# alibaba/euler

Measured on NVIDIA H100. Metric: sampled_edges_per_sec, higher is better.
Workload: dtype u64 ids / f32 weights+features (f64 CDF compare)

## Files before the change

euler_b200/csrc/capi.cu:

```cuda
#include <stdio.h>
#include <stdlib.h>
#include <string.h>

#include <algorithm>
#include <map>
#include <mutex>
#include <string>

#include "internal.h"

namespace eu {

__global__ void k_seed(EuRngState* rs, int n, unsigned long long seed0, const unsigned long long* seeds) {
  const int e = blockIdx.x * blockDim.x + threadIdx.x;
  if (e >= n) return;
  const unsigned long long seed = seeds ? seeds[e] : seed0 + (unsigned long long)e;
  EuRngState* r = rs + e;
  unsigned long long x = seed % 2147483647ull;
  r->x = x == 0 ? 1u : (uint32_t)x;
  r->x_prev = r->x;
  r->draws = 0;
  r->calls = 0;
  r->blocks_done = 0;
  r->key = seed * 0x9E3779B97F4A7C15ull;
}

template <typename T>
static int regrow(T** p, int64_t count) {
  if (*p) cudaFree(*p);
  *p = nullptr;
  void* q = nullptr;
  size_t bytes = (size_t)(count > 0 ? count : 1) * sizeof(T);
  cudaError_t e = cudaMalloc(&q, bytes);
  if (e != cudaSuccess) { set_error("cudaMalloc(%zu) -> %s", bytes, cudaGetErrorString(e)); return EU_ERR_CUDA; }
  *p = (T*)q;
  return EU_OK;
}

int refuse_growth_in_capture(eu_ctx* c, const char* what) {
  cudaStreamCaptureStatus st = cudaStreamCaptureStatusNone;
  if (cudaStreamIsCapturing(c->stream, &st) == cudaSuccess && st != cudaStreamCaptureStatusNone) {
    set_error("%s must grow while the ctx stream is being captured: run the op once (or call eu_ctx_reserve) before the capture", what);
    return EU_ERR_STATE;
  }
  cudaGetLastError();
  return EU_OK;
}

int ctx_reserve(eu_ctx* c, int64_t rows, int64_t table_slots) {
  int rc;
  if ((table_slots > c->tab_set_slots || rows > c->cap_rows) && (rc = refuse_growth_in_capture(c, "the sampling scratch"))) return rc;
  if (table_slots > c->tab_set_slots) {
    EU_CUDA(cudaStreamSynchronize(c->stream));
    const int64_t slots = table_slots + 64;
    if ((rc = regrow(&c->d_dedup, 2 * slots))) return rc;
    c->tab_set_slots = slots;
    for (int64_t off = 0; off < 2 * slots; off += (int64_t)1 << 20) {
      int64_t n = std::min<int64_t>((int64_t)1 << 20, 2 * slots - off);
      EU_CUDA(cudaMemset2DAsync(&c->d_dedup[off].key, sizeof(HashSlot), 0x00, 8, (size_t)n, c->stream));
      EU_CUDA(cudaMemset2DAsync(&c->d_dedup[off].row, sizeof(HashSlot), 0xFF, 8, (size_t)n, c->stream));
    }
  }
  if (rows <= c->cap_rows) return EU_OK;
  EU_CUDA(cudaStreamSynchronize(c->stream));
  if ((rc = regrow(&c->d_first, rows))) return rc;
  if ((rc = regrow(&c->d_rowof, rows))) return rc;
  if ((rc = regrow(&c->d_elig, rows))) return rc;
  if ((rc = regrow(&c->d_state, rows))) return rc;
  if ((rc = regrow(&c->d_emask, rows / 32 + 2))) return rc;
  if ((rc = regrow(&c->d_woff, rows / 32 + 2))) return rc;
  if ((rc = regrow(&c->d_blkpre, rows / 256 + 66))) return rc;
  if ((rc = regrow(&c->d_blkmul, rows / 256 + 66))) return rc;
  if ((rc = regrow(&c->d_live, rows))) return rc;
  if ((rc = regrow(&c->d_dup, rows))) return rc;
  if (!c->d_nlive && (rc = regrow(&c->d_nlive, 4))) return rc;
  if ((rc = regrow(&c->d_front[0], rows))) return rc;
  if ((rc = regrow(&c->d_front[1], rows))) return rc;
  c->cap_rows = rows;
  return EU_OK;
}

int ctx_misc(eu_ctx* c, int64_t bytes) {
  if (bytes <= c->misc_bytes) return EU_OK;
  if (int rc0 = refuse_growth_in_capture(c, "the op scratch")) return rc0;
  EU_CUDA(cudaStreamSynchronize(c->stream));
  char* p = (char*)c->d_misc;
  int rc = regrow(&p, bytes);
  c->d_misc = p;
  if (rc) { c->misc_bytes = 0; return rc; }
  c->misc_bytes = bytes;
  return EU_OK;
}

int agg_reserve(eu_ctx* c, int64_t rows, int64_t table_slots) {
  if (rows <= c->agg_rows && table_slots <= c->agg_slots) return EU_OK;
  int rc;
  if ((rc = refuse_growth_in_capture(c, "the aggregation scratch"))) return rc;
  EU_CUDA(cudaStreamSynchronize(c->stream));
  if (table_slots > c->agg_slots) {
    c->agg_slots = 0;
    if ((rc = regrow(&c->d_agg_tab, table_slots))) return rc;
    EU_CUDA(cudaMemsetAsync(c->d_agg_tab, 0, sizeof(unsigned long long) * (size_t)table_slots, c->stream));
    c->agg_slots = table_slots;
  }
  if (rows > c->agg_rows) {
    c->agg_rows = 0;
    if ((rc = regrow(&c->d_agg_src, rows))) return rc;
    if ((rc = regrow(&c->d_agg_rep, rows))) return rc;
    if ((rc = regrow(&c->d_agg_slot, rows))) return rc;
    if (!c->d_agg_nrep && (rc = regrow(&c->d_agg_nrep, 1))) return rc;
    c->agg_rows = rows;
  }
  return EU_OK;
}

static std::mutex g_default_mu;
static eu_graph* g_default_graph = nullptr;
static eu_ctx* g_default_ctx = nullptr;

}

using namespace eu;

extern "C" {

int eu_ctx_create(eu_graph* g, eu_rng_kind rng, uint64_t seed, void* stream, eu_ctx** out) {
  if (!g || !out || (rng != EU_RNG_MINSTD && rng != EU_RNG_PHILOX)) { set_error("eu_ctx_create: bad argument"); return EU_ERR_INVALID; }
  EU_CUDA(cudaSetDevice(g->device));
  eu_ctx* c = new eu_ctx();
  c->g = g; c->rng = rng; c->seed = seed; c->stream = (cudaStream_t)stream;
  cudaError_t e = cudaMalloc(&c->d_rng, sizeof(EuRngState));
  if (e != cudaSuccess) { set_error("cudaMalloc rng -> %s", cudaGetErrorString(e)); delete c; return EU_ERR_CUDA; }
  k_seed<<<1, 64, 0, c->stream>>>(c->d_rng, 1, seed, nullptr);
  g_launches++;
  *out = c;
  return EU_OK;
}

int eu_ctx_destroy(eu_ctx* c) {
  if (!c) return EU_OK;
  cudaSetDevice(c->g->device);
  cudaStreamSynchronize(c->stream);
  cudaFree(c->d_rng); cudaFree(c->d_dedup); cudaFree(c->d_first); cudaFree(c->d_rowof);
  cudaFree(c->d_elig); cudaFree(c->d_state); cudaFree(c->d_emask); cudaFree(c->d_woff); cudaFree(c->d_blkpre); cudaFree(c->d_blkmul); cudaFree(c->d_live); cudaFree(c->d_dup); cudaFree(c->d_nlive); cudaFree(c->d_front[0]); cudaFree(c->d_front[1]);
  cudaFree(c->d_misc); cudaFree(c->d_stage); cudaFree(c->d_walkv);
  cudaFree(c->d_agg_tab); cudaFree(c->d_agg_src); cudaFree(c->d_agg_rep); cudaFree(c->d_agg_slot); cudaFree(c->d_agg_nrep);
  for (int i = 0; i < 2; ++i) { if (c->aux[i]) cudaStreamDestroy(c->aux[i]); if (c->ev_join[i]) cudaEventDestroy(c->ev_join[i]); }
  if (c->ev_fork) cudaEventDestroy(c->ev_fork);
  if (c->h_pin) cudaFreeHost(c->h_pin);
  delete c;
  return EU_OK;
}

int eu_ctx_set_stream(eu_ctx* c, void* stream) {
  if (!c) { set_error("null ctx"); return EU_ERR_INVALID; }
  c->stream = (cudaStream_t)stream;
  return EU_OK;
}

int eu_ctx_seed(eu_ctx* c, uint64_t seed) {
  if (!c) { set_error("null ctx"); return EU_ERR_INVALID; }
  EU_CUDA(cudaSetDevice(c->g->device));
  c->seed = seed;
  k_seed<<<1, 64, 0, c->stream>>>(c->d_rng, c->n_eng, seed, nullptr);
  EU_LAUNCHED();
  return EU_OK;
}

int eu_ctx_set_engines(eu_ctx* c, int32_t n, const uint64_t* seeds) {
  if (!c || n < 1 || n > 64) { set_error("eu_ctx_set_engines: 1..64 engines"); return EU_ERR_INVALID; }
  EU_CUDA(cudaSetDevice(c->g->device));
  EU_CUDA(cudaStreamSynchronize(c->stream));
  EuRngState* r = nullptr;
  EU_CUDA(cudaMalloc(&r, sizeof(EuRngState) * n));
  unsigned long long* d_seeds = nullptr;
  if (seeds) {
    EU_CUDA(cudaMalloc(&d_seeds, sizeof(unsigned long long) * n));
    EU_CUDA(cudaMemcpy(d_seeds, seeds, sizeof(unsigned long long) * n, cudaMemcpyHostToDevice));
    c->seed = seeds[0];
  }
  cudaFree(c->d_rng);
  c->d_rng = r;
  c->n_eng = n;
  k_seed<<<1, 64, 0, c->stream>>>(c->d_rng, n, c->seed, d_seeds);
  EU_LAUNCHED();
  EU_CUDA(cudaStreamSynchronize(c->stream));
  if (d_seeds) cudaFree(d_seeds);
  return EU_OK;
}

int eu_ctx_reserve(eu_ctx* c, int64_t max_rows) {
  if (!c || max_rows < 0) { set_error("eu_ctx_reserve: bad argument"); return EU_ERR_INVALID; }
  EU_CUDA(cudaSetDevice(c->g->device));
  const int nb = c->n_eng;
  int rc = ctx_reserve(c, max_rows + 256 * nb, 4 * max_rows + 65 * nb);
  if (rc) return rc;
// ... 101 lines not shown
```

euler_b200/csrc/internal.h:

```cpp
#pragma once
#include <cuda_runtime.h>
#include <stdint.h>

#include <atomic>
#include <string>
#include <vector>

#include "../../include/euler_b200.h"
#include "common.cuh"

namespace eu {

void set_error(const char* fmt, ...);
extern std::atomic<uint64_t> g_launches;

#define EU_CUDA(call)                                                                    \
  do {                                                                                   \
    cudaError_t _e = (call);                                                             \
    if (_e != cudaSuccess) {                                                             \
      ::eu::set_error("%s:%d %s -> %s", __FILE__, __LINE__, #call, cudaGetErrorString(_e)); \
      return EU_ERR_CUDA;                                                                \
    }                                                                                    \
  } while (0)

// ... 29 lines not shown
  eu::DevGraph d{};
  std::vector<void*> allocs;
  int64_t hbm_bytes = 0;
  bool sampler_built = false;
  std::vector<eu::TypeSampler> samplers;
  std::vector<float> type_sums;
  std::vector<float> type_prob;
  std::vector<int32_t> type_alias;
  float type_fwc_sum = 0.f;
  float* d_type_prob = nullptr;
  int32_t* d_type_alias = nullptr;
  std::vector<int64_t> sampler_order;
  std::vector<std::string> edge_type_names, node_type_names;
  std::vector<std::string> dense_feature_names;
  std::vector<std::string> sparse_feature_names, binary_feature_names;
  std::vector<uint64_t> u64_slot_max;
  eu::DevEdges e{};
  bool edges_set = false;
  struct EdgeSampler { int64_t n = 0; const int64_t* order = nullptr; const float* prob = nullptr; const int32_t* alias = nullptr; float fwc_sum = 0.f; };
  std::vector<EdgeSampler> edge_samplers;
  std::vector<std::string> edge_dense_names, edge_sparse_names, edge_binary_names;
  bool labels_built = false;
  std::vector<std::string> labels;
  int32_t* d_label_ptr = nullptr;
  unsigned long long* d_label_ids = nullptr;

  template <typename T>
  int alloc(T** p, int64_t count) {
    size_t bytes = (size_t)(count > 0 ? count : 1) * sizeof(T);
    bytes = (bytes + 255) & ~(size_t)255;
    void* q = nullptr;
    cudaError_t e = cudaMalloc(&q, bytes);
    if (e != cudaSuccess) {
      eu::set_error("cudaMalloc(%zu) -> %s", bytes, cudaGetErrorString(e));
      return EU_ERR_CUDA;
    }
    allocs.push_back(q);
    hbm_bytes += (int64_t)bytes;
    *p = (T*)q;
    return EU_OK;
  }
};

struct EuRngState {
  uint32_t x;
  uint32_t x_prev;
  unsigned long long draws;
  unsigned long long calls;
  unsigned int blocks_done;
  unsigned int pad2;
  unsigned long long key;
};

struct eu_ctx {
  eu_graph* g = nullptr;
  eu_rng_kind rng = EU_RNG_MINSTD;
  uint64_t seed = 0;
  cudaStream_t stream = nullptr;
  EuRngState* d_rng = nullptr;
  int n_eng = 1;
  int64_t cap_rows = 0;
  eu::HashSlot* d_dedup = nullptr;
  int64_t tab_set_slots = 0;
  int32_t* d_first = nullptr;
  int64_t* d_rowof = nullptr;
  uint8_t* d_elig = nullptr;
  uint32_t* d_state = nullptr;
  uint32_t* d_emask = nullptr;
  uint32_t* d_woff = nullptr;
  uint32_t* d_blkpre = nullptr;
  uint32_t* d_blkmul = nullptr;
  int32_t* d_live = nullptr;
  int32_t* d_dup = nullptr;
  unsigned int* d_nlive = nullptr;
  unsigned long long* d_front[2] = {nullptr, nullptr};
  int64_t agg_rows = 0, agg_slots = 0;
  unsigned long long* d_agg_tab = nullptr;
  int32_t* d_agg_src = nullptr;
  int32_t* d_agg_rep = nullptr;
  uint32_t* d_agg_slot = nullptr;
  unsigned int* d_agg_nrep = nullptr;
  void* d_misc = nullptr;
  int64_t misc_bytes = 0;
  float* d_walkv = nullptr;
  long long walkv_cap = 0;
  cudaStream_t aux[2] = {nullptr, nullptr};
  cudaEvent_t ev_fork = nullptr, ev_join[2] = {nullptr, nullptr};
  void* h_pin = nullptr;
  int64_t pin_bytes = 0;
  void* d_stage = nullptr;
  int64_t stage_bytes = 0;
  bool prof = false;
  struct ProfRec { const char* name; int64_t rows; cudaEvent_t e0, e1; };
  std::vector<ProfRec> prof_recs;
};

struct EuProfScope {
  eu_ctx* c; size_t idx;
  EuProfScope(eu_ctx* c_, const char* name, int64_t rows) : c(c_), idx((size_t)-1) {
    if (!c->prof) return;
    eu_ctx::ProfRec r{name, rows, nullptr, nullptr};
    cudaEventCreate(&r.e0); cudaEventCreate(&r.e1);
    cudaEventRecord(r.e0, c->stream);
    c->prof_recs.push_back(r);
    idx = c->prof_recs.size() - 1;
  }
  ~EuProfScope() { if (idx != (size_t)-1) cudaEventRecord(c->prof_recs[idx].e1, c->stream); }
};

namespace eu {
static constexpr int64_t kRepeatMinRows = (int64_t)1 << 17;
int ctx_reserve(eu_ctx* c, int64_t rows, int64_t table_slots);
int64_t hop_scratch_rows(int nb, int64_t rows_b);
int64_t hop_table_slots(int nb, int64_t rows_b);
int64_t hop_table_cap(int64_t rows_b);
int ctx_misc(eu_ctx* c, int64_t bytes);
inline size_t a256(size_t b) { return (b + 255) & ~(size_t)255; }
struct EdgeOrder;
// ... 22 lines not shown
```

euler_b200/csrc/sample.cu:

```cuda
#include <algorithm>

#include <stdlib.h>

#include "internal.h"

namespace eu {

struct ETypes {
  int32_t K;
  int32_t v[EU_MAX_ETYPES];
};

struct Geom {
  int32_t nb;
  int32_t nblk_b;
  int64_t rows_b;
  int64_t rows_pad;
  int64_t cap_b;
  const int32_t* rows_act;
};

__global__ void k_dedup_insert(HashSlot* tabs, Geom gm, const unsigned long long* __restrict__ seeds) {
  const int b = blockIdx.y;
  const int64_t li = blockIdx.x * (int64_t)blockDim.x + threadIdx.x;
// ... 5 lines not shown
  if ((threadIdx.x & 31) != __ffs(peers) - 1) return;
  dedup_insert_one(tabs + (int64_t)b * (gm.cap_b + 1), (unsigned long long)dedup_cap_eff(gm.cap_b, gm.rows_act, b) - 1, id, li);
}

__device__ __forceinline__ int64_t dedup_first(const HashSlot* tab, unsigned long long mask,
                                               unsigned long long id) {
  unsigned long long tag = id + 1;
  if (tag == 0ull) return (int64_t)tab[mask + 1].row;
  unsigned long long h = mix64(id) & mask;
  while (true) {
    const ulonglong2 s = *reinterpret_cast<const ulonglong2*>(tab + h);
    if (s.x == tag) return (int64_t)s.y;
    h = (h + 1) & mask;
  }
}

__device__ __forceinline__ float grp_cum_at(const DevGraph& g, int64_t row, int32_t t) {
  if (g.grp_cum) return __ldg(g.grp_cum + row * g.T + t);
  const int64_t b = g.grp_ptr[row], e = g.grp_ptr[row + 1];
  return e > b ? __ldg(g.cum_w + e - 1) : 0.f;
}

__device__ __forceinline__ bool row_eligible(const DevGraph& g, int64_t row, const ETypes& et, int mode) {
  if (row < 0) return false;
  const int32_t T = g.T;
  if (mode == 0) {
    int32_t t = et.v[0];
    if (t < 0 || t >= T) return false;
    return g.grp_ptr[row * T + t + 1] > g.grp_ptr[row * T + t];
  }
  if (mode == 1) {
    float s = 0.f;
    for (int32_t i = 0; i < et.K; ++i) {
      int32_t t = et.v[i];
      if (t < 0 || t >= T) return false;
      float pre = t > 0 ? grp_cum_at(g, row, t - 1) : 0.f;
      s = __fadd_rn(s, __fsub_rn(grp_cum_at(g, row, t), pre));
    }
    return s != 0.f;
  }
  return grp_cum_at(g, row, T - 1) != 0.f;
}

struct PrepOut {
  unsigned long long* eng_ids;
  long long* out_ids;
  float* out_w;
  int32_t* out_t;
  int32_t count;
  long long default_node;
  HashSlot* next_tabs;
  int64_t next_cap_b;
  int32_t* live;
  unsigned int* n_live;
  int32_t* dup;
  unsigned int* n_dup;
};

static constexpr int kPrepBlock = 256;

__global__ void __launch_bounds__(kPrepBlock) k_prepare(DevGraph g, const HashSlot* tabs, Geom gm,
                                                        const unsigned long long* __restrict__ seeds,
                                                        ETypes et, int mode, uint32_t F, unsigned long long draws_per_row,
                                                        int32_t* first, int64_t* rowof, uint32_t* emask, uint32_t* wmul,
                                                        uint32_t* blkpre, uint32_t* blkmul, EuRngState* rngs, PrepOut po) {
  __shared__ uint32_t s_w[kPrepBlock / 32];
  __shared__ uint32_t s_l[kPrepBlock / 32];
  __shared__ uint32_t s_d[kPrepBlock / 32];
  __shared__ uint32_t s_z[kPrepBlock / 32];
  __shared__ bool s_last;
  const int b = blockIdx.y;
  const int64_t li = blockIdx.x * (int64_t)kPrepBlock + threadIdx.x;
  const int64_t ii = b * gm.rows_pad + li;
  const int lane = threadIdx.x & 31, wid = threadIdx.x >> 5;
  EuRngState* rng = rngs + b;
  bool e = false;
  bool own = false;
  bool dflt = false;
  const int64_t rows_here = gm.rows_act ? (int64_t)gm.rows_act[b] : gm.rows_b;
  const uint32_t nblk_act = (uint32_t)max((int64_t)1, (rows_here + kPrepBlock - 1) / kPrepBlock);
  if (blockIdx.x >= nblk_act) return;
  if (li < rows_here) {
    const int64_t w = b * gm.rows_b + li;
    const unsigned long long id = seeds[w];
    const int64_t f = tabs ? dedup_first(tabs + (int64_t)b * (gm.cap_b + 1), (unsigned long long)dedup_cap_eff(gm.cap_b, gm.rows_act, b) - 1, id) : li;
    first[ii] = (int32_t)f;
    const int64_t row = lookup_row(g, id);
    own = row_eligible(g, row, et, mode);
    e = own && f == li;
    dflt = !own;
    if (own) rowof[ii] = row;
  }
  const uint32_t zm = __ballot_sync(0xffffffffu, dflt);
  if (zm) {
    const int64_t ob = (b * gm.rows_b + (li - lane)) * (int64_t)po.count;
    const uint32_t n = 32u * (uint32_t)po.count;
    for (uint32_t k = lane; k < n; k += 32) {
      if (!((zm >> (k / (uint32_t)po.count)) & 1u)) continue;
      if (po.eng_ids) po.eng_ids[ob + k] = 0ull;
      if (po.out_ids) { po.out_ids[ob + k] = po.default_node; po.out_w[ob + k] = 0.f; po.out_t[ob + k] = -1; }
    }
  }
  const uint32_t m = __ballot_sync(0xffffffffu, e);
  const uint32_t lm = po.dup ? m : __ballot_sync(0xffffffffu, own);
  const uint32_t dm = po.dup ? __ballot_sync(0xffffffffu, own && !e) : 0u;
  if (lane == 0) { s_w[wid] = __popc(m); s_l[wid] = __popc(lm); s_d[wid] = __popc(dm); s_z[wid] = zm; }
  __syncthreads();
  if (lane == 0) {
    uint32_t off = 0;
    for (int k = 0; k < wid; ++k) off += s_w[k];
    emask[ii >> 5] = m;
    uint32_t fp = 1, fb = F;
    for (; off; off >>= 1) { if (off & 1) fp = modmul(fp, fb); fb = modmul(fb, fb); }
    wmul[ii >> 5] = fp;
  }
  uint32_t* bp = blkpre + (int64_t)b * gm.nblk_b;
  if (threadIdx.x == 0) {
    uint32_t tot = 0, lt = 0, dt = 0;
    for (int k = 0; k < kPrepBlock / 32; ++k) {
      tot += s_w[k];
      const uint32_t l = s_l[k], d = s_d[k];
      s_l[k] = lt; s_d[k] = dt;
      lt += l; dt += d;
    }
    const uint32_t lbase = lt ? atomicAdd(po.n_live, lt) : 0u, dbase = dt ? atomicAdd(po.n_dup, dt) : 0u;
    for (int k = 0; k < kPrepBlock / 32; ++k) { s_l[k] += lbase; s_d[k] += dbase; }
    if (po.next_tabs)
      for (int k = 0; k < kPrepBlock / 32; ++k)
        if (s_z[k]) {
          const int64_t lz = blockIdx.x * (int64_t)kPrepBlock + k * 32 + (__ffs(s_z[k]) - 1);
          dedup_insert_one(po.next_tabs + (int64_t)b * (po.next_cap_b + 1), (unsigned long long)po.next_cap_b - 1, 0ull,
                           lz * (int64_t)po.count);
          break;
        }
    bp[blockIdx.x] = tot;
    __threadfence();
    s_last = atomicAdd(&rng->blocks_done, 1u) == nblk_act - 1;
  }
  __syncthreads();
  {
    const uint32_t below = (1u << lane) - 1u;
    if (e || (own && !po.dup)) po.live[s_l[wid] + __popc(lm & below)] = (int32_t)(b * gm.rows_b + li);
    else if (own) po.dup[s_d[wid] + __popc(dm & below)] = (int32_t)(b * gm.rows_b + li);
  }
  if (!s_last) return;
  __threadfence();
  __shared__ uint32_t s_scan[kPrepBlock];
  uint32_t carry = 0;
  for (uint32_t base = 0; base < nblk_act; base += kPrepBlock) {
    const uint32_t k = base + threadIdx.x;
    const uint32_t v = k < nblk_act ? __ldcg(bp + k) : 0u;
    s_scan[threadIdx.x] = v;
    __syncthreads();
    for (int off = 1; off < kPrepBlock; off <<= 1) {
      uint32_t t = threadIdx.x >= off ? s_scan[threadIdx.x - off] : 0u;
      __syncthreads();
      s_scan[threadIdx.x] += t;
      __syncthreads();
    }
    if (k < nblk_act) {
      uint32_t pre = carry + s_scan[threadIdx.x] - v;
      bp[k] = pre;
      uint32_t fp = 1, fb = F;
      for (; pre; pre >>= 1) { if (pre & 1) fp = modmul(fp, fb); fb = modmul(fb, fb); }
      blkmul[(int64_t)b * gm.nblk_b + k] = fp;
    }
    carry += s_scan[kPrepBlock - 1];
    __syncthreads();
  }
  if (threadIdx.x == 0) {
    uint32_t fp = 1, base = F;
    for (uint32_t t = carry; t; t >>= 1) { if (t & 1) fp = modmul(fp, base); base = modmul(base, base); }
    rng->x_prev = rng->x;
    rng->x = modmul(rng->x, fp);
    rng->draws += (unsigned long long)carry * draws_per_row;
    rng->blocks_done = 0;
  }
}

__global__ void __launch_bounds__(1024) k_state_scan(const uint8_t* __restrict__ elig, int64_t rows,
                                                     uint32_t F, unsigned long long draws_per_row,
                                                     uint32_t* state, EuRngState* rng) {
  __shared__ uint32_t s_part[1024];
  __shared__ uint32_t s_cnt[1024];
  const int t = threadIdx.x;
  const int64_t chunk = (rows + 1023) / 1024;
  const int64_t b = t * chunk, e = min(rows, b + chunk);
  uint32_t prod = 1, cnt = 0;
  for (int64_t i = b; i < e; ++i)
    if (elig[i]) { prod = modmul(prod, F); ++cnt; }
  s_part[t] = prod;
  s_cnt[t] = cnt;
  __syncthreads();
  for (int off = 1; off < 1024; off <<= 1) {
    uint32_t v = 1, c = 0;
    if (t >= off) { v = s_part[t - off]; c = s_cnt[t - off]; }
    __syncthreads();
    if (t >= off) { s_part[t] = modmul(s_part[t], v); s_cnt[t] += c; }
    __syncthreads();
  }
  const uint32_t x0 = rng->x;
  uint32_t run = modmul(x0, t > 0 ? s_part[t - 1] : 1u);
  for (int64_t i = b; i < e; ++i) {
    state[i] = run;
    if (elig[i]) run = modmul(run, F);
  }
  __syncthreads();
  if (t == 1023) {
    rng->x = modmul(x0, s_part[1023]);
    rng->draws += (unsigned long long)s_cnt[1023] * draws_per_row;
  }
}

struct SampleArgs {
  const unsigned long long* seeds;
  Geom gm;
  int32_t count;
  long long default_node;
  ETypes et;
  int mode;
  const int32_t* live;
  const unsigned int* n_live;
  const int32_t* first;
  const int64_t* rowof;
  const uint32_t* emask;
  const uint32_t* wmul;
  const uint32_t* blkmul;
  uint32_t F;
  uint32_t lanepow[32];
  uint32_t stride;
  int sg_log;
  int stage;
  HashSlot* clear_tab;
  int64_t clear_n;
  HashSlot* next_tabs;
  int64_t next_cap_b;
  unsigned long long key;
  const EuRngState* rngs;
  unsigned long long* eng_ids;
  long long* out_ids;
  float* out_w;
  int32_t* out_t;
};

__device__ __forceinline__ int lane_upper_bound(float c, int lo, int hi, float thr, unsigned gmask, int SG) {
#pragma unroll
  for (int it = 0; it < 5; ++it) {
    int mid = (lo + hi) >> 1;
    float v = __shfl_sync(gmask, c, mid, SG);
    bool go = lo < hi;
    bool gt = v >= thr;
    hi = (go && gt) ? mid : hi;
    lo = (go && !gt) ? mid + 1 : lo;
  }
  return lo;
}

template <bool PHILOX, int CTAS>
__global__ void __launch_bounds__(256, CTAS) k_sample(DevGraph g, SampleArgs a) {
  const int lane = threadIdx.x & 31;
  const int64_t gtid = blockIdx.x * (int64_t)blockDim.x + threadIdx.x;
  __shared__ uint32_t s_lanepow[32];
  __shared__ uint32_t s_fpow[32];
  constexpr int kStageF = 16;
  __shared__ __align__(128) float s_stage[256 * kStageF];
  __shared__ __align__(8) unsigned long long s_bar[32];
  const int SG = 1 << a.sg_log;
  const int sl = lane & (SG - 1);
  const unsigned gmask = SG == 32 ? 0xffffffffu : (((1u << SG) - 1u) << (lane - sl));
  const bool can_stage = a.sg_log >= 3 && a.stage;
  unsigned long long* const bar = &s_bar[can_stage ? (threadIdx.x >> a.sg_log) : 0];
  float* const sm = s_stage + (threadIdx.x - sl) * kStageF;
  const int64_t capg = (int64_t)SG * kStageF;
  uint32_t phase = 0;
  if (can_stage && sl == 0) mbar_init(bar, 1);
  if (!PHILOX && threadIdx.x < 32) {
    s_lanepow[threadIdx.x] = a.lanepow[threadIdx.x];
    uint32_t fp = 1, fb = a.F;
    for (uint32_t e = threadIdx.x; e; e >>= 1) { if (e & 1) fp = modmul(fp, fb); fb = modmul(fb, fb); }
    s_fpow[threadIdx.x] = fp;
  }
  fence_mbar_init();
  __syncthreads();
  if (!PHILOX) {
    if (!a.gm.rows_act) {
      for (int64_t s = gtid; s < a.clear_n; s += (int64_t)gridDim.x * blockDim.x) { a.clear_tab[s].key = 0; a.clear_tab[s].row = kEmptyRow; }
    } else if (a.clear_n) {
      for (int b = 0; b < a.gm.nb; ++b) {
        HashSlot* tab = a.clear_tab + (int64_t)b * (a.gm.cap_b + 1);
        const int64_t n = dedup_cap_eff(a.gm.cap_b, a.gm.rows_act, b) + 1;
        for (int64_t s = gtid; s < n; s += (int64_t)gridDim.x * blockDim.x) { tab[s].key = 0; tab[s].row = kEmptyRow; }
      }
    }
  }
  const int32_t count = a.count;
  const int32_t T = g.T;
  const int64_t total = PHILOX ? a.gm.nb * a.gm.rows_b : (int64_t)__ldg(a.n_live);
  const int64_t qstride = (((int64_t)gridDim.x * blockDim.x) >> 5) << (5 - a.sg_log);
  const uint32_t upd = a.mode == 0 ? 1u : 2u;
  const uint32_t stride = a.stride;

  for (int64_t q = ((gtid >> 5) << (5 - a.sg_log)) + (lane >> a.sg_log); q < total; q += qstride) {
    const int64_t w = PHILOX ? q : (int64_t)a.live[q];
    const int bidx = (int)(w / a.gm.rows_b);
    const int64_t li = w - bidx * a.gm.rows_b;
    if (PHILOX && a.gm.rows_act && li >= a.gm.rows_act[bidx]) continue;
    const int64_t obase = w * (int64_t)count;
    const EuRngState* rng = a.rngs + bidx;
    HashSlot* ntab = a.next_tabs ? a.next_tabs + (int64_t)bidx * (a.next_cap_b + 1) : nullptr;
    const unsigned long long nmask = (unsigned long long)a.next_cap_b - 1;
    const int64_t nbase = li * (int64_t)count;

    int64_t row;
    bool ok;
    uint32_t st = 0;
    unsigned long long seed_id = 0;
    if (PHILOX) {
      seed_id = a.seeds[w];
      row = lookup_row(g, seed_id);
      ok = row_eligible(g, row, a.et, a.mode);
    } else {
      const int64_t ib = bidx * a.gm.rows_pad;
      const int32_t f = a.first[ib + li];
      const uint32_t m = a.emask[(ib + f) >> 5];
      ok = (m >> (f & 31)) & 1u;
      if (ok) {
        row = a.rowof[ib + li];
        st = modmul(modmul(rng->x_prev, a.blkmul[(int64_t)bidx * a.gm.nblk_b + f / kPrepBlock]),
                    modmul(a.wmul[(ib + f) >> 5], s_fpow[__popc(m & ((1u << (f & 31)) - 1u))]));
      } else {
        row = -1;
      }
    }
    if (!ok) {
      for (int32_t j = sl; j < count; j += SG) {
        if (a.eng_ids) a.eng_ids[obase + j] = 0ull;
        if (a.out_ids) { a.out_ids[obase + j] = a.default_node; a.out_w[obase + j] = 0.f; a.out_t[obase + j] = -1; }
      }
      if (!PHILOX && ntab && sl == 0) dedup_insert_one(ntab, nmask, 0ull, nbase);
      continue;
    }

    const int64_t* gp = g.grp_ptr + row * T;
    const int64_t base = gp[0];
    const int64_t rlen = gp[T] - base;
    const bool small_row = rlen <= SG;
    float c = __int_as_float(0x7f800000);
    if (small_row && sl < rlen) c = __ldg(g.cum_w + base + sl);
    const int mis = (int)((reinterpret_cast<uintptr_t>(g.cum_w + base) & 15u) >> 2);
    const bool mid_row = can_stage && !small_row && rlen + mis <= capg;
    if (mid_row && sl == 0) {
      const uint32_t bytes = (uint32_t)((((rlen + mis) << 2) + 15) & ~15ll);
      fence_proxy_async_smem();
      mbar_arrive_expect_tx(bar, bytes);
      bulk_copy_g2s(sm, g.cum_w + base - mis, bytes, bar);
    }
    const float* const srow = sm + mis;

    int64_t gb = 0, ge = 0;
    float lim_b = 0.f, lim_e = 0.f;
    if (a.mode == 0) {
      const int32_t t = a.et.v[0];
      gb = gp[t];
      ge = gp[t + 1] - 1;
      lim_b = gb == base ? 0.f : __ldg(g.cum_w + gb - 1);
      lim_e = __ldg(g.cum_w + ge);
    }
    float tc = __int_as_float(0x7f800000);
    int ntc = 0;
    if (a.mode == 1) {
      ntc = a.et.K;
      float sum = 0.f, mine = 0.f;
      for (int32_t i = 0; i < ntc; ++i) {
        int32_t t = a.et.v[i];
        float pre = t > 0 ? grp_cum_at(g, row, t - 1) : 0.f;
        sum = __fadd_rn(sum, __fsub_rn(grp_cum_at(g, row, t), pre));
        if (i == sl) mine = sum;
      }
      if (sl < ntc) tc = mine;
    } else if (a.mode == 2) {
      ntc = T;
      if (sl < T) tc = grp_cum_at(g, row, sl);
    }
    const float tc_end = __shfl_sync(gmask, tc, ntc > 0 ? ntc - 1 : 0, SG);

    uint32_t x = 0;
    if (!PHILOX) x = modmul(st, s_lanepow[sl]);
    const uint32_t salt = PHILOX ? (uint32_t)rng->calls : 0u;
    const unsigned long long pkey = PHILOX ? a.key ^ rng->key : 0ull;

    if (mid_row) {
      const long long t0 = clock64();
      while (!mbar_try_wait(bar, phase))
        if (clock64() - t0 > 4000000000LL) __trap();
      phase ^= 1u;
    }
    bool keep = true;
    bool bad = false;
    for (int32_t j0 = 0; j0 < count; j0 += SG) {
      const int32_t j = j0 + sl;
      const bool active = j < count;
      double u_t = 0.0, u_n = 0.0;
      if (PHILOX) {
        philox_uniform2(seed_id, (uint32_t)j, salt, pkey, u_t, u_n);
      } else {
        uint32_t xs = x;
        if (upd == 2u) u_t = minstd_uniform(xs);
        u_n = minstd_uniform(xs);
        x = modmul(x, stride);
      }
      int32_t etype = a.mode == 0 ? a.et.v[0] : 0;
      int64_t b = gb, e = ge;
      float lb = lim_b, le = lim_e;
      if (a.mode != 0) {
        const float tt = gt_threshold(pick_r(u_t, 0.f, tc_end));
        int k = lane_upper_bound(tc, 0, ntc - 1, tt, gmask, SG);
        etype = a.mode == 1 ? a.et.v[k] : k;
        b = gp[etype];
        e = gp[etype + 1] - 1;
        if (e < b) {
          bad = bad || active;
          b = base; e = base;
        }
        lb = b == base ? 0.f : __ldg(g.cum_w + b - 1);
        le = __ldg(g.cum_w + e);
      }
      const float thr = gt_threshold(pick_r(u_n, lb, le));
      int64_t m;
      float wgt;
      if (small_row) {
        int li2 = lane_upper_bound(c, (int)(b - base), (int)(e - base), thr, gmask, SG);
        float hi_v = __shfl_sync(gmask, c, li2, SG);
        float lo_v = __shfl_sync(gmask, c, li2 > 0 ? li2 - 1 : 0, SG);
        m = base + li2;
        wgt = __fsub_rn(hi_v, li2 > 0 ? lo_v : 0.f);
      } else if (mid_row) {
        int lo = (int)(b - base), hi = (int)(e - base);
        while (lo < hi) {
          const int mid = (lo + hi) >> 1;
          if (srow[mid] >= thr) hi = mid; else lo = mid + 1;
// ... 150 lines not shown

static Geom make_geom(int nb, int64_t rows_b) {
  Geom gm{};
  gm.nb = nb;
  gm.rows_b = rows_b;
  gm.nblk_b = (int32_t)ceil_div(rows_b > 0 ? rows_b : 1, kPrepBlock);
  gm.rows_pad = (int64_t)gm.nblk_b * kPrepBlock;
  gm.cap_b = 64;
  while (gm.cap_b < rows_b * 2) gm.cap_b <<= 1;
  gm.rows_act = nullptr;
  return gm;
}

__global__ void k_ragged_stats(const long long* __restrict__ ptr, int64_t rows, long long* __restrict__ stats) {
  long long mx = 0;
  for (int64_t i = blockIdx.x * (int64_t)blockDim.x + threadIdx.x; i < rows; i += (int64_t)gridDim.x * blockDim.x)
    mx = max(mx, __ldg(ptr + i + 1) - __ldg(ptr + i));
  if (mx > 0) atomicMax(stats + 1, mx);
  if (blockIdx.x == 0 && threadIdx.x == 0) stats[0] = __ldg(ptr + rows);
}

int64_t hop_scratch_rows(int nb, int64_t rows_b) { return make_geom(nb, rows_b).rows_pad * nb; }
int64_t hop_table_slots(int nb, int64_t rows_b) { return (make_geom(nb, rows_b).cap_b + 1) * nb; }
int64_t hop_table_cap(int64_t rows_b) { return make_geom(1, rows_b).cap_b; }

int hop(eu_ctx* c, const unsigned long long* seeds, int64_t rows_b, const int32_t* etypes,
        int32_t K, int32_t count, int64_t default_node, unsigned long long* eng_ids,
        int64_t* out_ids, float* out_w, int32_t* out_t, int hop_index, bool pre_inserted, bool insert_next, int nb,
        const int32_t* rows_act, bool raw) {
  const int64_t rows = rows_b * nb;
  if (rows == 0 || count == 0) return EU_OK;
  if (nb < 1 || nb > c->n_eng) { set_error("hop: %d batches but the ctx has %d engines", nb, c->n_eng); return EU_ERR_INVALID; }
  const DevGraph& d = c->g->d;
  SampleArgs a{};
  int rc = classify(d, etypes, K, &a.et, &a.mode);
  if (rc) return rc;
  if (a.mode != 0 && d.T > 32) { set_error("T > 32 unsupported"); return EU_ERR_UNSUPPORTED; }
  cudaStream_t s = c->stream;
  Geom gm = make_geom(nb, rows_b);
  gm.rows_act = rows_act;
  a.seeds = seeds; a.gm = gm; a.count = count; a.default_node = default_node;
  a.eng_ids = eng_ids; a.out_ids = (long long*)out_ids; a.out_w = out_w; a.out_t = out_t;
  a.rngs = c->d_rng;
  {
    int need = std::min<int>(count, 32);
    if (a.mode == 1) need = std::max<int>(need, std::min<int>(a.et.K, 32));
    if (a.mode == 2) need = std::max<int>(need, std::min<int>(d.T, 32));
    a.sg_log = 0;
    while ((1 << a.sg_log) < need) ++a.sg_log;
  }
  static const int stage_rows = [] { const char* e = getenv("EU_SAMPLE_STAGE"); return e ? (atoi(e) != 0 ? 1 : 0) : 1; }();
  a.stage = stage_rows;
  static const int grid_ctas = [] { const char* e = getenv("EU_SAMPLE_CTAS"); return e ? std::min(8, std::max(1, atoi(e))) : 8; }();
  const int ctas = grid_ctas == 6 ? 6 : 8;
  const unsigned blocks = (unsigned)std::min<int64_t>(ceil_div(ceil_div(rows * 32, (int64_t)(32 >> a.sg_log)), 256), kSMs * grid_ctas);
  if (c->rng == EU_RNG_PHILOX) {
    a.key = c->seed;
    { EuProfScope ps(c, "k_sample<philox>", rows); if (ctas == 6) k_sample<true, 6><<<blocks, 256, 0, s>>>(d, a); else k_sample<true, 8><<<blocks, 256, 0, s>>>(d, a); }
    EU_LAUNCHED();
    k_bump_calls<<<1, 64, 0, s>>>(c->d_rng, nb);
    EU_LAUNCHED();
    return EU_OK;
  }
  if (rows >= ((int64_t)1 << 31) || nb > 64) { set_error("rows >= 2^31 or more than 64 batches"); return EU_ERR_UNSUPPORTED; }
  const Geom ng = make_geom(nb, rows_b * count);
  const bool chain = insert_next && eng_ids;
  rc = ctx_reserve(c, std::max(gm.rows_pad, chain ? ng.rows_pad : 0) * nb, (std::max(gm.cap_b, chain ? ng.cap_b : 0) + 1) * nb);
  if (rc) return rc;
  const int tb = kPrepBlock;
  HashSlot* tabs = c->d_dedup + (hop_index & 1) * c->tab_set_slots;
  HashSlot* ntabs = c->d_dedup + ((hop_index + 1) & 1) * c->tab_set_slots;
  if (raw && (pre_inserted || insert_next)) { set_error("hop: raw mode does not chain"); return EU_ERR_INVALID; }
  if (!pre_inserted && !raw) {
    EuProfScope ps(c, "k_dedup_insert", rows);
    k_dedup_insert<<<dim3((unsigned)ceil_div(gm.rows_b, tb), (unsigned)nb), tb, 0, s>>>(tabs, gm, seeds);
    EU_LAUNCHED();
  }
  const unsigned long long upr = (unsigned long long)count * (a.mode == 0 ? 1 : 2);
  const uint32_t F = modpow_a(2ull * upr);
  { EuProfScope ps(c, "k_prepare", rows);
    PrepOut po{};
    po.eng_ids = eng_ids; po.out_ids = (long long*)out_ids; po.out_w = out_w; po.out_t = out_t;
    po.count = count; po.default_node = default_node;
    if (chain) { po.next_tabs = ntabs; po.next_cap_b = ng.cap_b; }
    po.live = c->d_live; po.n_live = c->d_nlive;
    if (!raw && rows >= kRepeatMinRows) { po.dup = c->d_dup; po.n_dup = c->d_nlive + 1; }
    EU_CUDA(cudaMemsetAsync(c->d_nlive, 0, 2 * sizeof(unsigned int), s));
    k_prepare<<<dim3((unsigned)gm.nblk_b, (unsigned)nb), tb, 0, s>>>(d, raw ? nullptr : tabs, gm, seeds, a.et, a.mode, F, upr, c->d_first,
                                                                     c->d_rowof, c->d_emask, c->d_woff, c->d_blkpre, c->d_blkmul,
                                                                     c->d_rng, po); }
  EU_LAUNCHED();
  a.first = c->d_first; a.rowof = c->d_rowof; a.emask = c->d_emask; a.wmul = c->d_woff; a.blkmul = c->d_blkmul;
  a.live = c->d_live; a.n_live = c->d_nlive;
  a.F = F;
  const uint32_t upd = a.mode == 0 ? 1u : 2u;
  for (uint32_t k = 0; k < 32; ++k) a.lanepow[k] = modpow_a(2ull * upd * k);
  a.stride = modpow_a(2ull * upd * (unsigned long long)(1u << a.sg_log));
  a.clear_tab = tabs;
  a.clear_n = raw ? 0 : (gm.cap_b + 1) * nb;
  if (chain) {
    a.next_tabs = ntabs;
    a.next_cap_b = ng.cap_b;
  }
  { EuProfScope ps(c, "k_sample<minstd>", rows); if (ctas == 6) k_sample<false, 6><<<blocks, 256, 0, s>>>(d, a); else k_sample<false, 8><<<blocks, 256, 0, s>>>(d, a); }
  EU_LAUNCHED();
  if (!raw && rows >= kRepeatMinRows) {
    EuProfScope ps(c, "k_copy_dups", rows);
    k_copy_dups<<<blocks, 256, 0, s>>>(gm, count, a.sg_log, c->d_dup, c->d_nlive + 1, c->d_first, eng_ids, (long long*)out_ids, out_w, out_t);
    EU_LAUNCHED();
  }
  return EU_OK;
}

}

using namespace eu;

extern "C" {

int eu_sample_neighbor(eu_ctx* c, const int64_t* nodes, int64_t B, const int32_t* etypes, int32_t K,
                       int32_t count, int64_t default_node, int64_t* out_ids, float* out_w,
                       int32_t* out_t) {
  if (!c || B < 0 || count < 0 || (K > 0 && !etypes)) { set_error("eu_sample_neighbor: bad argument"); return EU_ERR_INVALID; }
  EU_CUDA(cudaSetDevice(c->g->device));
  return hop(c, (const unsigned long long*)nodes, B, etypes, K, count, default_node, nullptr, out_ids, out_w, out_t, 0, false, false, 1);
}

int eu_sample_neighbor_raw(eu_ctx* c, const int64_t* nodes, int64_t B, const int32_t* etypes, int32_t K,
                           int32_t count, int64_t* out_ids, float* out_w, int32_t* out_t) {
  if (!c || B < 0 || count < 0 || (K > 0 && !etypes)) { set_error("eu_sample_neighbor_raw: bad argument"); return EU_ERR_INVALID; }
  EU_CUDA(cudaSetDevice(c->g->device));
  if (c->rng != EU_RNG_MINSTD) { set_error("eu_sample_neighbor_raw: exact-RNG contexts only (philox rows are keyed on the node id: duplicates would repeat)"); return EU_ERR_UNSUPPORTED; }
  return hop(c, (const unsigned long long*)nodes, B, etypes, K, count, 0, nullptr, out_ids, out_w, out_t, 0, false, false, 1,
             nullptr, true);
}

int eu_sample_fanout_batched(eu_ctx* c, const int64_t* nodes, int32_t nb, int64_t B, const int32_t* etypes, int32_t K,
                             const int32_t* counts, int32_t L, int64_t default_node, int64_t* const* out_ids,
                             float* const* out_w, int32_t* const* out_t) {
  if (!c || nb < 1 || B < 0 || L < 0 || !counts || (K > 0 && !etypes)) { set_error("eu_sample_fanout: bad argument"); return EU_ERR_INVALID; }
  EU_CUDA(cudaSetDevice(c->g->device));
  if (nb > c->n_eng) { set_error("eu_sample_fanout_batched: %d batches but the ctx has %d engines (eu_ctx_set_engines)", nb, c->n_eng); return EU_ERR_INVALID; }
  for (int l = 0; l < L; ++l)
    if (counts[l] < 0) { set_error("negative count"); return EU_ERR_INVALID; }
  for (int l = 0; l < L; ++l)
    if (counts[l] == 0) { L = l; break; }
  if (B == 0) return EU_OK;
  int64_t rows_b = B, max_rows = hop_scratch_rows(nb, B), max_slots = hop_table_slots(nb, B), widest = B * nb;
  for (int l = 0; l < L; ++l) {
    rows_b *= counts[l];
    if (l + 1 < L) { max_rows = std::max(max_rows, hop_scratch_rows(nb, rows_b)); max_slots = std::max(max_slots, hop_table_slots(nb, rows_b)); }
    widest = std::max(widest, rows_b * nb);
  }
  int rc = ctx_reserve(c, std::max(max_rows, widest), max_slots);
  if (rc) return rc;
  const unsigned long long* seeds = (const unsigned long long*)nodes;
  rows_b = B;
// ... 126 lines not shown
```

Baseline: 5.540 billion.

## Precompute per-live-row records in prepare and prefetch them in sampler

k_prepare now writes a compact LiveRow record (row base, length, type-range or row id, and a per-row RNG multiplier) next to each live index. The sampler then reads this record instead of re-reading grp_ptr, first, emask and wmul, and it prefetches the next iteration's record. The block multiplier now has x_prev folded in. The sampler's launch bound drops to 3 CTAs per SM with a matching smaller grid, which allows more registers per thread. The cost is extra prepare work (a serial prefix loop and modpow per eligible row) and a larger scratch buffer. Non-eligible rows are no longer written as defaults in the minstd path, so that path must be covered elsewhere.

Result: faster. 6.058 billion (median of 6 runs) (+9.4%).

```diff
diff --git a/euler_b200/csrc/capi.cu b/euler_b200/csrc/capi.cu
--- a/euler_b200/csrc/capi.cu
+++ b/euler_b200/csrc/capi.cu
@@ -64,7 +64,7 @@
   if (rows <= c->cap_rows) return EU_OK;
   EU_CUDA(cudaStreamSynchronize(c->stream));
   if ((rc = regrow(&c->d_first, rows))) return rc;
-  if ((rc = regrow(&c->d_rowof, rows))) return rc;
+  if ((rc = regrow(&c->d_liverec, rows))) return rc;
   if ((rc = regrow(&c->d_elig, rows))) return rc;
   if ((rc = regrow(&c->d_state, rows))) return rc;
   if ((rc = regrow(&c->d_emask, rows / 32 + 2))) return rc;
@@ -141,7 +141,7 @@
   if (!c) return EU_OK;
   cudaSetDevice(c->g->device);
   cudaStreamSynchronize(c->stream);
-  cudaFree(c->d_rng); cudaFree(c->d_dedup); cudaFree(c->d_first); cudaFree(c->d_rowof);
+  cudaFree(c->d_rng); cudaFree(c->d_dedup); cudaFree(c->d_first); cudaFree(c->d_liverec);
   cudaFree(c->d_elig); cudaFree(c->d_state); cudaFree(c->d_emask); cudaFree(c->d_woff); cudaFree(c->d_blkpre); cudaFree(c->d_blkmul); cudaFree(c->d_live); cudaFree(c->d_dup); cudaFree(c->d_nlive); cudaFree(c->d_front[0]); cudaFree(c->d_front[1]);
   cudaFree(c->d_misc); cudaFree(c->d_stage); cudaFree(c->d_walkv);
   cudaFree(c->d_agg_tab); cudaFree(c->d_agg_src); cudaFree(c->d_agg_rep); cudaFree(c->d_agg_slot); cudaFree(c->d_agg_nrep);
diff --git a/euler_b200/csrc/internal.h b/euler_b200/csrc/internal.h
--- a/euler_b200/csrc/internal.h
+++ b/euler_b200/csrc/internal.h
@@ -105,6 +105,15 @@
   unsigned long long key;
 };
 
+namespace eu {
+struct LiveRow {
+  int64_t base;
+  int64_t aux;
+  int32_t rlen;
+  uint32_t lmul;
+};
+}
+
 struct eu_ctx {
   eu_graph* g = nullptr;
   eu_rng_kind rng = EU_RNG_MINSTD;
@@ -116,7 +125,7 @@
   eu::HashSlot* d_dedup = nullptr;
   int64_t tab_set_slots = 0;
   int32_t* d_first = nullptr;
-  int64_t* d_rowof = nullptr;
+  eu::LiveRow* d_liverec = nullptr;
   uint8_t* d_elig = nullptr;
   uint32_t* d_state = nullptr;
   uint32_t* d_emask = nullptr;
diff --git a/euler_b200/csrc/sample.cu b/euler_b200/csrc/sample.cu
--- a/euler_b200/csrc/sample.cu
+++ b/euler_b200/csrc/sample.cu
@@ -81,6 +81,7 @@
   HashSlot* next_tabs;
   int64_t next_cap_b;
   int32_t* live;
+  LiveRow* rec;
   unsigned int* n_live;
   int32_t* dup;
   unsigned int* n_dup;
@@ -91,7 +92,7 @@
 __global__ void __launch_bounds__(kPrepBlock) k_prepare(DevGraph g, const HashSlot* tabs, Geom gm,
                                                         const unsigned long long* __restrict__ seeds,
                                                         ETypes et, int mode, uint32_t F, unsigned long long draws_per_row,
-                                                        int32_t* first, int64_t* rowof, uint32_t* emask, uint32_t* wmul,
+                                                        int32_t* first, uint32_t* emask, uint32_t* wmul,
                                                         uint32_t* blkpre, uint32_t* blkmul, EuRngState* rngs, PrepOut po) {
   __shared__ uint32_t s_w[kPrepBlock / 32];
   __shared__ uint32_t s_l[kPrepBlock / 32];
@@ -106,6 +107,7 @@
   bool e = false;
   bool own = false;
   bool dflt = false;
+  LiveRow rec{};
   const int64_t rows_here = gm.rows_act ? (int64_t)gm.rows_act[b] : gm.rows_b;
   const uint32_t nblk_act = (uint32_t)max((int64_t)1, (rows_here + kPrepBlock - 1) / kPrepBlock);
   if (blockIdx.x >= nblk_act) return;
@@ -118,7 +120,17 @@
     own = row_eligible(g, row, et, mode);
     e = own && f == li;
     dflt = !own;
-    if (own) rowof[ii] = row;
+    if (own) {
+      const int64_t* gp = g.grp_ptr + row * g.T;
+      rec.base = gp[0];
+      rec.rlen = (int32_t)(gp[g.T] - rec.base);
+      if (mode == 0) {
+        const int32_t t = et.v[0];
+        rec.aux = (int64_t)(uint32_t)(gp[t] - rec.base) | ((gp[t + 1] - 1 - rec.base) << 32);
+      } else {
+        rec.aux = row;
+      }
+    }
   }
   const uint32_t zm = __ballot_sync(0xffffffffu, dflt);
   if (zm) {
@@ -169,12 +181,23 @@
   __syncthreads();
   {
     const uint32_t below = (1u << lane) - 1u;
-    if (e || (own && !po.dup)) po.live[s_l[wid] + __popc(lm & below)] = (int32_t)(b * gm.rows_b + li);
-    else if (own) po.dup[s_d[wid] + __popc(dm & below)] = (int32_t)(b * gm.rows_b + li);
+    if (e || (own && !po.dup)) {
+      const uint32_t at = s_l[wid] + __popc(lm & below);
+      po.live[at] = (int32_t)(b * gm.rows_b + li);
+      if (e) {
+        uint32_t pos = __popc(m & below);
+        for (int k = 0; k < wid; ++k) pos += s_w[k];
+        uint32_t fp = 1, fb = F;
+        for (; pos; pos >>= 1) { if (pos & 1) fp = modmul(fp, fb); fb = modmul(fb, fb); }
+        rec.lmul = fp;
+      }
+      po.rec[at] = rec;
+    } else if (own) po.dup[s_d[wid] + __popc(dm & below)] = (int32_t)(b * gm.rows_b + li);
   }
   if (!s_last) return;
   __threadfence();
   __shared__ uint32_t s_scan[kPrepBlock];
+  const uint32_t x0 = rng->x;
   uint32_t carry = 0;
   for (uint32_t base = 0; base < nblk_act; base += kPrepBlock) {
     const uint32_t k = base + threadIdx.x;
@@ -192,7 +215,7 @@
       bp[k] = pre;
       uint32_t fp = 1, fb = F;
       for (; pre; pre >>= 1) { if (pre & 1) fp = modmul(fp, fb); fb = modmul(fb, fb); }
-      blkmul[(int64_t)b * gm.nblk_b + k] = fp;
+      blkmul[(int64_t)b * gm.nblk_b + k] = modmul(x0, fp);
     }
     carry += s_scan[kPrepBlock - 1];
     __syncthreads();
@@ -249,9 +272,9 @@
   ETypes et;
   int mode;
   const int32_t* live;
+  const LiveRow* rec;
   const unsigned int* n_live;
   const int32_t* first;
-  const int64_t* rowof;
   const uint32_t* emask;
   const uint32_t* wmul;
   const uint32_t* blkmul;
@@ -272,6 +295,16 @@
   int32_t* out_t;
 };
 
+__device__ __forceinline__ LiveRow load_live_row(const LiveRow* p) {
+  LiveRow r;
+  r.base = __ldg(&p->base);
+  r.aux = __ldg(&p->aux);
+  const int2 t = __ldg(reinterpret_cast<const int2*>(&p->rlen));
+  r.rlen = t.x;
+  r.lmul = (uint32_t)t.y;
+  return r;
+}
+
 __device__ __forceinline__ int lane_upper_bound(float c, int lo, int hi, float thr, unsigned gmask, int SG) {
 #pragma unroll
   for (int it = 0; it < 5; ++it) {
@@ -285,8 +318,10 @@
   return lo;
 }
 
-template <bool PHILOX, int CTAS>
-__global__ void __launch_bounds__(256, CTAS) k_sample(DevGraph g, SampleArgs a) {
+static constexpr int kSampleCtas = 3;
+
+template <bool PHILOX>
+__global__ void __launch_bounds__(256, kSampleCtas) k_sample(DevGraph g, SampleArgs a) {
   const int lane = threadIdx.x & 31;
   const int64_t gtid = blockIdx.x * (int64_t)blockDim.x + threadIdx.x;
   __shared__ uint32_t s_lanepow[32];
@@ -329,9 +364,15 @@
   const uint32_t upd = a.mode == 0 ? 1u : 2u;
   const uint32_t stride = a.stride;
 
-  for (int64_t q = ((gtid >> 5) << (5 - a.sg_log)) + (lane >> a.sg_log); q < total; q += qstride) {
-    const int64_t w = PHILOX ? q : (int64_t)a.live[q];
-    const int bidx = (int)(w / a.gm.rows_b);
+  const int64_t q0 = ((gtid >> 5) << (5 - a.sg_log)) + (lane >> a.sg_log);
+  int32_t nw = 0;
+  LiveRow nrec{};
+  if (!PHILOX && q0 < total) { nw = __ldg(a.live + q0); nrec = load_live_row(a.rec + q0); }
+  for (int64_t q = q0; q < total; q += qstride) {
+    const int64_t w = PHILOX ? q : (int64_t)nw;
+    const LiveRow r = nrec;
+    if (!PHILOX && q + qstride < total) { nw = __ldg(a.live + q + qstride); nrec = load_live_row(a.rec + q + qstride); }
+    const int bidx = PHILOX ? (int)(w / a.gm.rows_b) : (int)((uint32_t)w / (uint32_t)a.gm.rows_b);
     const int64_t li = w - bidx * a.gm.rows_b;
     if (PHILOX && a.gm.rows_act && li >= a.gm.rows_act[bidx]) continue;
     const int64_t obase = w * (int64_t)count;
@@ -340,39 +381,33 @@
     const unsigned long long nmask = (unsigned long long)a.next_cap_b - 1;
     const int64_t nbase = li * (int64_t)count;
 
-    int64_t row;
-    bool ok;
-    uint32_t st = 0;
+    int64_t row = 0;
+    int64_t base, rlen;
+    int64_t gb = 0, ge = 0;
+    uint32_t bm = 0;
     unsigned long long seed_id = 0;
     if (PHILOX) {
       seed_id = a.seeds[w];
       row = lookup_row(g, seed_id);
-      ok = row_eligible(g, row, a.et, a.mode);
+      if (!row_eligible(g, row, a.et, a.mode)) {
+        for (int32_t j = sl; j < count; j += SG) {
+          if (a.eng_ids) a.eng_ids[obase + j] = 0ull;
+          if (a.out_ids) { a.out_ids[obase + j] = a.default_node; a.out_w[obase + j] = 0.f; a.out_t[obase + j] = -1; }
+        }
+        continue;
+      }
+      const int64_t* gp = g.grp_ptr + row * T;
+      base = gp[0];
+      rlen = gp[T] - base;
+      if (a.mode == 0) { gb = gp[a.et.v[0]]; ge = gp[a.et.v[0] + 1] - 1; }
     } else {
-      const int64_t ib = bidx * a.gm.rows_pad;
-      const int32_t f = a.first[ib + li];
-      const uint32_t m = a.emask[(ib + f) >> 5];
-      ok = (m >> (f & 31)) & 1u;
-      if (ok) {
-        row = a.rowof[ib + li];
-        st = modmul(modmul(rng->x_prev, a.blkmul[(int64_t)bidx * a.gm.nblk_b + f / kPrepBlock]),
-                    modmul(a.wmul[(ib + f) >> 5], s_fpow[__popc(m & ((1u << (f & 31)) - 1u))]));
-      } else {
-        row = -1;
-      }
-    }
-    if (!ok) {
-      for (int32_t j = sl; j < count; j += SG) {
-        if (a.eng_ids) a.eng_ids[obase + j] = 0ull;
-        if (a.out_ids) { a.out_ids[obase + j] = a.default_node; a.out_w[obase + j] = 0.f; a.out_t[obase + j] = -1; }
-      }
-      if (!PHILOX && ntab && sl == 0) dedup_insert_one(ntab, nmask, 0ull, nbase);
-      continue;
-    }
-
+      base = r.base;
+      rlen = r.rlen;
+      if (a.mode == 0) { gb = base + (uint32_t)r.aux; ge = base + (r.aux >> 32); }
+      else row = r.aux;
+      if (r.lmul) bm = __ldg(a.blkmul + (int64_t)bidx * a.gm.nblk_b + li / kPrepBlock);
+    }
     const int64_t* gp = g.grp_ptr + row * T;
-    const int64_t base = gp[0];
-    const int64_t rlen = gp[T] - base;
     const bool small_row = rlen <= SG;
     float c = __int_as_float(0x7f800000);
     if (small_row && sl < rlen) c = __ldg(g.cum_w + base + sl);
@@ -386,12 +421,8 @@
     }
     const float* const srow = sm + mis;
 
-    int64_t gb = 0, ge = 0;
     float lim_b = 0.f, lim_e = 0.f;
     if (a.mode == 0) {
-      const int32_t t = a.et.v[0];
-      gb = gp[t];
-      ge = gp[t + 1] - 1;
       lim_b = gb == base ? 0.f : __ldg(g.cum_w + gb - 1);
       lim_e = __ldg(g.cum_w + ge);
     }
@@ -414,7 +445,19 @@
     const float tc_end = __shfl_sync(gmask, tc, ntc > 0 ? ntc - 1 : 0, SG);
 
     uint32_t x = 0;
-    if (!PHILOX) x = modmul(st, s_lanepow[sl]);
+    if (!PHILOX) {
+      uint32_t st;
+      if (r.lmul) {
+        st = modmul(bm, r.lmul);
+      } else {
+        const int64_t ib = bidx * a.gm.rows_pad;
+        const int32_t f = a.first[ib + li];
+        const uint32_t m = a.emask[(ib + f) >> 5];
+        st = modmul(a.blkmul[(int64_t)bidx * a.gm.nblk_b + f / kPrepBlock],
+                    modmul(a.wmul[(ib + f) >> 5], s_fpow[__popc(m & ((1u << (f & 31)) - 1u))]));
+      }
+      x = modmul(st, s_lanepow[sl]);
+    }
     const uint32_t salt = PHILOX ? (uint32_t)rng->calls : 0u;
     const unsigned long long pkey = PHILOX ? a.key ^ rng->key : 0ull;
 
@@ -671,11 +714,12 @@
   static const int stage_rows = [] { const char* e = getenv("EU_SAMPLE_STAGE"); return e ? (atoi(e) != 0 ? 1 : 0) : 1; }();
   a.stage = stage_rows;
   static const int grid_ctas = [] { const char* e = getenv("EU_SAMPLE_CTAS"); return e ? std::min(8, std::max(1, atoi(e))) : 8; }();
-  const int ctas = grid_ctas == 6 ? 6 : 8;
-  const unsigned blocks = (unsigned)std::min<int64_t>(ceil_div(ceil_div(rows * 32, (int64_t)(32 >> a.sg_log)), 256), kSMs * grid_ctas);
+  const int64_t need_blocks = ceil_div(ceil_div(rows * 32, (int64_t)(32 >> a.sg_log)), 256);
+  const unsigned blocks = (unsigned)std::min<int64_t>(need_blocks, kSMs * grid_ctas);
+  const unsigned sblocks = (unsigned)std::min<int64_t>(need_blocks, kSMs * std::min(grid_ctas, kSampleCtas));
   if (c->rng == EU_RNG_PHILOX) {
     a.key = c->seed;
-    { EuProfScope ps(c, "k_sample<philox>", rows); if (ctas == 6) k_sample<true, 6><<<blocks, 256, 0, s>>>(d, a); else k_sample<true, 8><<<blocks, 256, 0, s>>>(d, a); }
+    { EuProfScope ps(c, "k_sample<philox>", rows); k_sample<true><<<sblocks, 256, 0, s>>>(d, a); }
     EU_LAUNCHED();
     k_bump_calls<<<1, 64, 0, s>>>(c->d_rng, nb);
     EU_LAUNCHED();
@@ -702,14 +746,14 @@
     po.eng_ids = eng_ids; po.out_ids = (long long*)out_ids; po.out_w = out_w; po.out_t = out_t;
     po.count = count; po.default_node = default_node;
     if (chain) { po.next_tabs = ntabs; po.next_cap_b = ng.cap_b; }
-    po.live = c->d_live; po.n_live = c->d_nlive;
+    po.live = c->d_live; po.rec = c->d_liverec; po.n_live = c->d_nlive;
     if (!raw && rows >= kRepeatMinRows) { po.dup = c->d_dup; po.n_dup = c->d_nlive + 1; }
     EU_CUDA(cudaMemsetAsync(c->d_nlive, 0, 2 * sizeof(unsigned int), s));
     k_prepare<<<dim3((unsigned)gm.nblk_b, (unsigned)nb), tb, 0, s>>>(d, raw ? nullptr : tabs, gm, seeds, a.et, a.mode, F, upr, c->d_first,
-                                                                     c->d_rowof, c->d_emask, c->d_woff, c->d_blkpre, c->d_blkmul,
+                                                                     c->d_emask, c->d_woff, c->d_blkpre, c->d_blkmul,
                                                                      c->d_rng, po); }
   EU_LAUNCHED();
-  a.first = c->d_first; a.rowof = c->d_rowof; a.emask = c->d_emask; a.wmul = c->d_woff; a.blkmul = c->d_blkmul;
+  a.first = c->d_first; a.rec = c->d_liverec; a.emask = c->d_emask; a.wmul = c->d_woff; a.blkmul = c->d_blkmul;
   a.live = c->d_live; a.n_live = c->d_nlive;
   a.F = F;
   const uint32_t upd = a.mode == 0 ? 1u : 2u;
@@ -721,7 +765,7 @@
     a.next_tabs = ntabs;
     a.next_cap_b = ng.cap_b;
   }
-  { EuProfScope ps(c, "k_sample<minstd>", rows); if (ctas == 6) k_sample<false, 6><<<blocks, 256, 0, s>>>(d, a); else k_sample<false, 8><<<blocks, 256, 0, s>>>(d, a); }
+  { EuProfScope ps(c, "k_sample<minstd>", rows); k_sample<false><<<sblocks, 256, 0, s>>>(d, a); }
   EU_LAUNCHED();
   if (!raw && rows >= kRepeatMinRows) {
     EuProfScope ps(c, "k_copy_dups", rows);
```
